# alibaba/open-simulator

Measured on AMD Instinct MI355X. Metric: capacity-plan scenarios/sec (10k pods x ~1k nodes), higher is better.
Workload: dtype u8 score table + u32 (gcd-normalised int64 quantities) + f64 (BalancedAllocation); 1 GPU; BASELINE config 3: 10000 pods x 488..1511 nodes, 1024 node counts x 4 pod orders = 4096 scenarios (4096 per GPU); scenarios_per_gpu=4096, pods=10000, node_pool=1512, kernel=score_table

## Files before the change

__graft_entry__.py:

```python
import os
import subprocess
import sys

ROOT = os.path.dirname(os.path.abspath(__file__))
if ROOT not in sys.path:
    sys.path.insert(0, ROOT)

CSRC = os.path.join(ROOT, "open-simulator_amd", "csrc")
HIP_SOURCES = ["simon_hip.hip", "simon_group.hip", "simon_narrow.hip", "simon_fast.hip", "simon_table.hip", "simon_table_spread.hip", "simon_table_spread2.hip", "simon_table_team4.hip", "simon_table_team4z.hip", "simon_table_rest.hip", "simon_table_rest2.hip", "simon_table_rs.hip", "simon_table_rsz.hip", "simon_table_cls4.hip", "simon_table_lds.hip", "simon_table_restlds.hip", "simon_image.hip", "simon_subset.hip", "simon_wide.hip", "simon_wide_local.hip", "simon_wide_explain.hip"]
HIP_HEADERS = ["simon_device.h", "simon_wide.h", "simon_table.h", "simon_subset.h", "simon_table_assume.inc", os.path.join(ROOT, "include", "simon_hip.h")]
EXTRA_DEPS = {**{f"simon_table_team{n}.hip": ["simon_table.hip"] for n in (4,)}, "simon_table_spread.hip": ["simon_table.hip"], "simon_table_spread2.hip": ["simon_table.hip"], "simon_table_rest.hip": ["simon_table.hip"], "simon_table_rest2.hip": ["simon_table.hip"], "simon_table_rs.hip": ["simon_table.hip"], "simon_table_rsz.hip": ["simon_table.hip"], "simon_table_team4z.hip": ["simon_table.hip"], "simon_table_cls4.hip": ["simon_table.hip"], "simon_table_lds.hip": ["simon_table.hip"], "simon_table_restlds.hip": ["simon_table.hip"], "simon_image.hip": ["simon_table.hip"],
              "simon_wide_local.hip": ["simon_wide.hip"], "simon_wide_explain.hip": ["simon_wide.hip"]}
HIPCC_FLAGS = ["--offload-arch=gfx950", "-O3", "-std=c++17", "-ffp-contract=off", "-fPIC"]


def _stale(target, deps):
    if not os.path.exists(target):
        return True
    t = os.path.getmtime(target)
    return any(os.path.getmtime(d) > t for d in deps)


def _isa_path(src):
    return os.path.join(ROOT, "build", "isa", os.path.basename(src)[:-4] + ".s")


def _spill_scan(hipcc, srcs, hdrs) -> None:
    os.makedirs(os.path.join(ROOT, "build", "isa"), exist_ok=True)
    outs, jobs = [], []
    for src in srcs:
        out = _isa_path(src)
        outs.append(out)
        if _stale(out, [src] + hdrs + [os.path.join(CSRC, d) for d in EXTRA_DEPS.get(os.path.basename(src), [])]):
            jobs.append((src, subprocess.Popen([hipcc, *HIPCC_FLAGS, "--cuda-device-only", "-S", "-o", out, src], stderr=subprocess.DEVNULL)))
    for src, job in jobs:
        if job.wait() != 0:
            raise RuntimeError(f"hipcc -S failed on {src}")
    sys.path.insert(0, os.path.join(ROOT, "profiles"))
    import spill_scan
    bad = []
    for out in outs:
        bad += [(os.path.basename(out),) + f for f in spill_scan.scan(out)[1]]
    if bad:
# ... 68 lines not shown
```

open-simulator_amd/csrc/simon_table.hip:

```cpp
#include "simon_table.h"

#include <algorithm>
#include <type_traits>

#ifdef SIMON_TABLE_PROFILE
#define TPROF_DECL unsigned long long tp_prev = __builtin_readcyclecounter(), tp_acc[24] = {0}; tp_acc[22] = tp_prev - tp_pro0; tp_acc[23] = tp_pro2;
#define TPROF_PROLOGUE_BEGIN const unsigned long long tp_pro0 = __builtin_readcyclecounter(); unsigned long long tp_pro2 = 0;
#define TPROF_TABLE_PASS_BEGIN tp_pro2 = __builtin_readcyclecounter()
#define TPROF_TABLE_PASS_END do { asm volatile("s_waitcnt vmcnt(0) lgkmcnt(0)" ::: "memory"); tp_pro2 = __builtin_readcyclecounter() - tp_pro2; } while (0)
#define TPROF(i) do { const unsigned long long t_ = __builtin_readcyclecounter(); tp_acc[i] += t_ - tp_prev; tp_prev = t_; } while (0)
#define TPROF_WAIT_LDS asm volatile("s_waitcnt lgkmcnt(0)" ::: "memory")
#define TPROF_WAIT_MEM asm volatile("s_waitcnt vmcnt(0)" ::: "memory")
#else
#define TPROF_DECL
#define TPROF_PROLOGUE_BEGIN
#define TPROF_TABLE_PASS_BEGIN do { } while (0)
#define TPROF_TABLE_PASS_END do { } while (0)
#define TPROF(i) do { } while (0)
#define TPROF_WAIT_LDS do { } while (0)
#define TPROF_WAIT_MEM do { } while (0)
#endif

namespace simon {

// ... 252 lines not shown
    const int32_t* __restrict__ orders, const int32_t* __restrict__ perm, const unsigned long long* __restrict__ ws_off,
    int32_t* __restrict__ place_step, unsigned char* ws, const TableScalars sc) {
    GPtr<const TableCold> const cold = gp(cold_);
    GPtr<const int32_t> __restrict__ const ncls = gp(cold->ncls);
    GPtr<const int32_t> __restrict__ const cls_off = gp(cold->cls_off); GPtr<const int32_t> __restrict__ const clsprefix = gp(cold->clsprefix);
    GPtr<const int32_t> __restrict__ const a_pods = gp(cold->a_pods); GPtr<const uint32_t> __restrict__ const i_rq_cpu = gp(cold->i_rq_cpu);
    GPtr<const uint32_t> __restrict__ const i_rq_mem = gp(cold->i_rq_mem); GPtr<const uint32_t> __restrict__ const i_nz_cpu = gp(cold->i_nz_cpu);
    GPtr<const uint32_t> __restrict__ const i_nz_mem = gp(cold->i_nz_mem); GPtr<const int32_t> __restrict__ const i_npods = gp(cold->i_npods);
    const SigRow* __restrict__ const sigs = cold->sigs; const ShapeRow* __restrict__ const shapes = cold->shapes;
    const ScenarioDesc* __restrict__ const scen = cold->scen; GPtr<const uint64_t> __restrict__ const static_mask = gp(cold->static_mask);
    GPtr<const int32_t> __restrict__ const simon_raw = gp(cold->simon_raw);
    extern __shared__ __attribute__((aligned(16))) unsigned char smem[];
    const int Cn = sc.Cn, Cp = sc.Cp, P = sc.P, K = sc.K;
    constexpr int UB = COARSE ? 6 : 4;
    constexpr int UNIT = 1 << UB;
    constexpr unsigned UMASK = UNIT - 1;
    constexpr int KB = COARSE ? 13 : 12;
    constexpr unsigned PMASK = (1u << KB) - 1u;
    static_assert(!REST || COARSE, "the REST path is built on the two-level layout");
    constexpr bool kCls4 = CN2 && !REST && !SPREAD;
#ifdef SIMON_REST_CNT_HBM
    constexpr bool CNT_LDS = !COARSE;
#else
    constexpr bool CNT_LDS = (!COARSE || REST) && !kCls4;
#endif
#ifdef SIMON_TIE_SPECULATE
    constexpr bool TIE_FIRST = false;
#else
    constexpr bool TIE_FIRST = REST || MANY;
#endif
    constexpr bool kStraight = !REST && !SPREAD && !MANY;
    static_assert(!(kStraight && TIE_FIRST), "the straight-line cycle defines the winner's class and record index behind the assume's loads: nothing ahead of them may read dstar / res");
    static_assert(!kStraight || NW == 1, "team mode is SPREAD: a straight-line instantiation has no helper waves");
    constexpr bool kSharedPro = kSharedPrologueTU && !COARSE && !REST && !SPREAD && !MANY && !kCls4 && !RANKED && !LDSWS && NW == 1;
    static_assert(!MANY || (KQ == 2 && COARSE && !CN2 && !LDSX), "MANY = groups of 128 signatures on the two-level layout (since round 6 also under the REST select: its rows and counters are indexed by signature already)");
    constexpr int NG = MANY ? 2 : 0;
    static_assert(!SPREAD || COARSE, "SPREAD is built on the two-level layout");
    constexpr bool RS = REST && SPREAD;
    static_assert(!RS || (!LDSX && !CN2), "REST && SPREAD: <= 64 classes");
    static_assert(!(SPREAD && MANY) || NBQ == 2, "SPREAD with more than 128 signatures: the two-blocks-per-lane instantiations only");
    static_assert(NW == 1 || SPREAD, "team mode exists for the SPREAD instantiations");
    static_assert(!CN2 || (SPREAD && !MANY && !REST) || (REST && !LDSX && !SPREAD) || (!REST && !SPREAD && !COARSE && !MANY && !LDSWS), "CN2 = two node classes per lane in spread_select (<= 128 signatures) or in rest_select (rows in HBM); without rows and walks: 129 .. 256 classes on the one-level layout (simon_table_cls4.hip)");
    constexpr int TABMAX = CN2 ? kSpreadTabMax2 : kSpreadTabMax;
    const TCarve cv = tcarve(K, sc.ni_max, Cn, COARSE, REST, SPREAD ? (sc.NZK | ((sc.static_tables & kStSpreadAff) ? 0x100 : 0) | (NW > 1 ? 0x200 : 0) | (CN2 ? 0x400 : 0)) : -1, kCls4);
    const int TH = SPREAD ? sc.TH : 0, TZ = SPREAD ? sc.TZ : 0, NZK = SPREAD ? sc.NZK : 0;
    signed char* s_zdom = (signed char*)(smem + cv.zdom);
    unsigned short* s_stash = (unsigned short*)(smem + cv.stash);
    int* s_tabi = (int*)(smem + cv.tabi);
    int* s_tab = (int*)(smem + cv.tab);
    int* s_tot = NW > 1 ? (int*)(smem + cv.tab2) : s_tab;
    int* s_xch = (int*)(smem + cv.xch);
    const int M = REST ? sc.M : 0, G = REST ? sc.G : 0, X = REST ? sc.X : 0, NZ = REST ? sc.NZ : 0;
    const int nbp = cv.nbp;
    unsigned short* s_sn = (unsigned short*)(smem + cv.sn);
    int* s_cnt = (int*)(smem + cv.cnt);
    const ShapeRow* s_shape = (const ShapeRow*)(smem + cv.shape);
    auto shape_of = [&](int d) -> ShapeRow {
        if constexpr (kCls4) {
            const double* r = (const double*)(smem + cv.shape) + 4 * d;
            return ShapeRow{r[0], r[1], r[2], r[3], 100.0 * r[2], 100.0 * r[3]};
        } else return s_shape[d];
    };
    int* s_seg = (int*)(smem + cv.seg);
    int* s_tmp = (int*)(smem + cv.tmp);
    int2* s_ext = (int2*)(smem + cv.ext);

// ... 302 lines not shown
    if constexpr (SPREAD) {
        for (int i = tid; i < (NZK > 0 ? NZK : 1) * Cn; i += TT) s_zdom[i] = NZK > 0 ? gp(cold->cls_zdom)[i] : (signed char)0;
        for (size_t i = tid; i < ((size_t)TH * ni + 3) / 4; i += TT) ((unsigned*)g_hrow)[i] = 0u;
        for (int i = tid; i < TZ * 16; i += TT) g_zcnt[i] = 0u;
        for (int i = tid; i < TH; i += TT) g_hmax[i] = 0;
    }
    asm volatile("s_waitcnt vmcnt(0)" ::: "memory");
    if constexpr (NW > 1 || kCls4) __threadfence();
    __syncthreads();
    if constexpr (NW > 1) __threadfence();

    int kk[KQ];
    bool kvalid[KQ];
    double my_req_c[KQ], my_req_m[KQ], my_nz_c[KQ], my_nz_m[KQ];
    bool my_zero[KQ];
    int my_tc[KQ];
    unsigned my_add_c[KQ], my_add_m[KQ], my_addz_c[KQ], my_addz_m[KQ], koff[KQ];
    unsigned my_greq[KQ];
    int my_gnum[KQ];
    unsigned my_dirty = 0;
#pragma unroll
    for (int q = 0; q < KQ; ++q) {
        kvalid[q] = lane + 64 * q < K;
        kk[q] = kvalid[q] ? lane + 64 * q : 0;
        const SigRow r = sigs[kk[q]];
        my_req_c[q] = r.req_c; my_req_m[q] = r.req_m; my_nz_c[q] = r.nz_c; my_nz_m[q] = r.nz_m;
        my_zero[q] = r.flags & 1u;
        if constexpr (kCls4) my_tc[q] = r.cls;
        my_greq[q] = (unsigned)r.pad[0]; my_gnum[q] = kvalid[q] ? r.pad[1] : 0;
        my_add_c[q] = (unsigned)r.req_c; my_add_m[q] = (unsigned)r.req_m;
        my_addz_c[q] = (unsigned)r.nz_c; my_addz_m[q] = (unsigned)r.nz_m;
        koff[q] = (unsigned)kk[q] * KS;
    }
    for (int j = 0; j * 64 + lane < K; ++j) my_dirty |= 1u << j;
    int cb[NBQ], bcls[NBQ], binfo[NBQ];
#pragma unroll
    for (int q = 0; q < NBQ; ++q) {
        const int b = q * 64 + lane;
        cb[q] = (((int)(PMASK >> UB)) - b) << UB;
        bcls[q] = class_of_pos(b < nun ? b * UNIT : 0);
        binfo[q] = (cls_off[bcls[q]] - s_seg[bcls[q]] + 8192) | (bcls[q] << 16);
    }

    auto winner_info = [&](int bw) -> int {
        const int l = bw & 63, h = bw >> 6;
        int info = __builtin_amdgcn_readlane(binfo[0], l);
        if (NBQ > 1) { const int i1 = __builtin_amdgcn_readlane(binfo[NBQ > 1 ? 1 : 0], l); info = h == 1 ? i1 : info; }
        if (NBQ > 2) {
            const int i2 = __builtin_amdgcn_readlane(binfo[NBQ > 2 ? 2 : 0], l), i3 = __builtin_amdgcn_readlane(binfo[NBQ > 3 ? 3 : 0], l);
            info = h == 2 ? i2 : h == 3 ? i3 : info;
        }
        return info;
    };

    auto img_base = [&](GPtr<const TableCold> cc) -> size_t {
        return (size_t)__builtin_amdgcn_readfirstlane(gp(cc->img_slot)[s]) * (size_t)cc->img_stride;
    };
    auto class_term = [&](bool inb, int rawc, int c, int dd) -> int {
        const int lo = wave_min_i32(inb ? rawc : 0x7fffffff);
        const int hi = wave_max_i32(inb ? rawc : (int)0x80000000);
        const int range = hi >= lo ? hi - lo : 0;
        const double rr = range ? 1.0 / (double)range : 0.0;
        int term = (inb && range) ? 2 * (int)__builtin_fma((double)(rawc - lo) * 100.0, rr, 0.5 * rr) : 0;
        GPtr<const TableCold> cc = cold;
        asm volatile("" : "+s"(cc));
        if (sc.static_tables & kStNa) {
            const int v = gp(cc->na_raw)[c * Cn + dd];
            const int mx = wave_max_i32(inb ? v : 0);
            const double r = mx ? 1.0 / (double)mx : 0.0;
            term += (inb && mx) ? (int)__builtin_fma((double)v * 100.0, r, 0.5 * r) : 0;
        }
        if (sc.static_tables & kStTt) {
            const int v = gp(cc->tt_raw)[c * Cn + dd];
            const int mx = wave_max_i32(inb ? v : 0);
            const double r = mx ? 1.0 / (double)mx : 0.0;
            term += inb ? (mx ? 100 - (int)__builtin_fma((double)v * 100.0, r, 0.5 * r) : 100) : 0;
        }
        if (sc.static_tables & kStAdd) term += inb ? gp(cc->add_raw)[c * Cn + dd] : 0;
        if (sc.static_tables & kStImg) term += inb ? (int)gp(cc->img)[img_base(cc) + c * Cn + dd] : 0;
        return term;
    };
    auto class_term2 = [&](bool in0, bool in1, int raw0, int raw1, int c, int d0, int d1, int& t0, int& t1) {
        const int lo = min(wave_min_i32(in0 ? raw0 : 0x7fffffff), wave_min_i32(in1 ? raw1 : 0x7fffffff));
        const int hi = max(wave_max_i32(in0 ? raw0 : (int)0x80000000), wave_max_i32(in1 ? raw1 : (int)0x80000000));
        const int range = hi >= lo ? hi - lo : 0;
        const double rr = range ? 1.0 / (double)range : 0.0;
// ... 929 lines not shown
            const int zd = s_zdom[zst * Cn + dstar];
            L.on = L.on && zd >= 0;
            L.old = g_zcnt[rowt * 16 + (zd >= 0 ? zd : 0)];
        } else {
            L.on = false;
        }
        return L;
    };
    auto spread_count_store = [&](const SpreadLoads& L, int pstar, int dstar, int spv, int spt, int soft_n, int match_n) {
        const int e = lane - soft_n;
        if (e < 0 || e >= match_n || !L.on) return;
        const unsigned mult = ((unsigned)spv >> 16) & 0xFFu;
        const int kindt = spt & 3, rowt = (spt >> 2) & 0x3FFF, zst = (spt >> 16) & 7;
        const unsigned nv = L.old + mult;
        if (kindt == 1) {
            g_hrow[(size_t)rowt * ni + (unsigned)pstar] = (unsigned char)nv;
            if (nv > L.mx) g_hmax[rowt] = (unsigned char)nv;
        } else {
            g_zcnt[rowt * 16 + s_zdom[zst * Cn + dstar]] = nv;
        }
    };

    int unsched = 0;
    int32_t* __restrict__ place = place_step ? place_step + (size_t)s * P : nullptr;

    auto load_chunk = [&](int i0) -> int4 {
        const int idx = i0 + lane;
        if (idx >= P) return make_int4((int)0x80000000, -1, 0x7fffffff, 0);
        const PodRowC r = pods[order[idx]];
        const bool gated_out = segd ? (r.gate >= 0 && gp(cold->rk_rank)[(size_t)s * (size_t)cold->N + r.gate] >= n) : r.gate >= n;
        const bool special = gated_out || r.preset != -1;
        return make_int4(r.sigcls | (special ? (int)0x80000000 : 0), r.preset, r.gate, r.rest);
    };
    int4 nxt = load_chunk(0);
    auto load_spw = [&](int i0) -> int {
        if constexpr (RS) { const int idx = i0 + lane; return idx < P ? gp(cold->sp_word)[order[idx]] : 0; }
        else return 0;
    };
    int nxt_sw = load_spw(0);
    uint4 pos_c = make_uint4(SIMON_POSC(0), SIMON_POSC(1), SIMON_POSC(2), SIMON_POSC(3));
    asm volatile("" : "+v"(pos_c.x), "+v"(pos_c.y), "+v"(pos_c.z), "+v"(pos_c.w));

    for (int i0 = 0; i0 < P; i0 += 64) {
        const int4 cur = nxt;
        nxt = load_chunk(i0 + 64);
        const int cur_sw = nxt_sw;
        if constexpr (RS) nxt_sw = load_spw(i0 + 64);
        int steps = P - i0 < 64 ? P - i0 : 64;
        if constexpr (kStraight) asm volatile("" : "+s"(steps));
        int plreg = -2;
        for (int il = 0; il < steps; ++il) {
        TPROF(0);
        const int pk = __builtin_amdgcn_readlane(cur.x, il);
        const int r_sig = pk & 0x3FF, r_cls = (pk >> 10) & 0x1FFFFF;
        const int rw = (REST || SPREAD) ? __builtin_amdgcn_readlane(cur.w, il) : 0;
        const int sw = RS ? __builtin_amdgcn_readlane(cur_sw, il) : rw;
        const int sp_soft = SPREAD ? (sw & 7) : 0, sp_match = SPREAD ? ((sw >> 3) & 127) : 0, sp_ipa = SPREAD ? ((sw >> 10) & 7) : 0, sp_hard = SPREAD ? ((sw >> 13) & 3) : 0;
        int spv = 0;
        int spt = 0;
        if (SPREAD && __builtin_expect(sw != 0, 0) && lane < sp_soft + sp_match + sp_ipa + sp_hard) {
            const int2 spe = ldg_i2(gp(cold->sp_ent) + (((unsigned)sw >> 15) + lane));
            spv = spe.x; spt = spe.y;
        }
        const int r_gs = REST ? (rw & 63) - 1 : -1, r_xs = REST ? ((rw >> 6) & 63) - 1 : -1, r_nrows = REST ? (rw >> 12) & 63 : 0;
        int rowv = 0;
        if (REST && lane < r_nrows) rowv = gp(cold->xrows)[((unsigned)rw >> 18) + lane];
        unsigned rtv = 0;
        if (REST && AFF && lane < r_nrows && ((unsigned)rowv >> 31)) rtv = g_rowtot[(unsigned)rowv & 0xFFFFu];

        const uint4* const sel_tab = (const uint4*)kSel;
        auto assume = [&](const bool scanned, const bool bound, int& pstar, int& dstar, int& res, const unsigned top, const unsigned (&m16q)[NBQ], const unsigned (&e16q)[NBQ]) __attribute__((always_inline)) {
            if constexpr (kStraight) {
#include "simon_table_assume.inc"
            }
        };
        int res, pstar = -1, dstar = 0;
        unsigned top = 0, m16q[NBQ], e16q[NBQ];
        bool scanned = false, bound = false;
        const bool spread_pod = SPREAD && pk >= 0 && (sp_soft | sp_ipa | sp_hard) != 0;
        if (!lead) {
            res = -2;
        } else if (__builtin_expect(pk < 0, 0)) {
            const int r_preset = __builtin_amdgcn_readlane(cur.y, il), r_gate = __builtin_amdgcn_readlane(cur.z, il);
            GPtr<const TableCold> cc = cold;
            asm volatile("" : "+s"(cc));
            if (segd ? (r_gate >= 0 && __builtin_amdgcn_readfirstlane(gp(cc->rk_rank)[(size_t)s * (size_t)cc->N + r_gate]) >= n) : r_gate >= n) {
                res = -2;
            } else if (r_preset >= 0) {
                bound = true;
                dstar = __builtin_amdgcn_readfirstlane(gp(cc->ncls)[r_preset]);
                const int rk = __builtin_amdgcn_readfirstlane(ranked ? gp(cc->rk_pos)[(size_t)s * (size_t)cc->N + r_preset] : gp(cc->rank)[r_preset]);
                pstar = __builtin_amdgcn_readfirstlane(s_seg[dstar]) + rk;
                res = __builtin_amdgcn_readfirstlane(gp(cc->cls_off)[dstar]) + rk;
            } else {
                const int pin = -2 - r_preset;
                res = -1;
                if (HAS_PIN && (segd ? __builtin_amdgcn_readfirstlane(gp(cc->rk_rank)[(size_t)s * (size_t)cc->N + pin]) < n : pin < n)) {
                    const int dp = __builtin_amdgcn_readfirstlane(gp(cc->ncls)[pin]);
                    const int rk = __builtin_amdgcn_readfirstlane(ranked ? gp(cc->rk_pos)[(size_t)s * (size_t)cc->N + pin] : gp(cc->rank)[pin]);
                    const int pp = __builtin_amdgcn_readfirstlane(s_seg[dp]) + rk;
                    const unsigned char byte = g_tile[tile_blk((unsigned)(pp >> 4)) + (unsigned)r_sig * KS + (unsigned)(pp & 15)];
                    bool clear = true;
                    if (REST && rw != 0) clear = !((__builtin_amdgcn_readfirstlane(excluded(pp >> 4, r_nrows, rowv, r_gs, r_xs, aff_escape(r_nrows, rowv, rtv))) >> (pp & 15)) & 1u);
                    if (byte != 0 && clear) { res = __builtin_amdgcn_readfirstlane(gp(cc->cls_off)[dp]) + rk; pstar = pp; dstar = dp; }
                }
            }
            if constexpr (kStraight) {
                if (pstar >= 0) assume(false, bound, pstar, dstar, res, 0u, m16q, e16q);
            }
        } else if (REST && __builtin_expect(rw != 0, 0) && !(RS && spread_pod)) {
            pstar = rest_select(r_sig, r_cls, r_nrows, rowv, r_gs, r_xs, aff_escape(r_nrows, rowv, rtv), dstar, res);
            TPROF(10);
            if (pstar < 0) res = -1;
        } else if (spread_pod) {
            const int k = r_sig;
            const unsigned dq = (unsigned)__builtin_amdgcn_readlane((int)my_dirty, k & 63);
            if ((dq >> (k >> 6)) & 1u) {
                renormalise(k, r_cls);
                if (lane == (k & 63)) my_dirty &= ~(1u << (k >> 6));
            }
            if constexpr (NW == 1) {
                if constexpr (RS) pstar = spread_select(k, r_cls, sp_soft, sp_match, sp_ipa, sp_hard, spv, spt, dstar, res, r_nrows, rowv, r_gs, r_xs, aff_escape(r_nrows, rowv, rtv));
                else pstar = spread_select(k, r_cls, sp_soft, sp_match, sp_ipa, sp_hard, spv, spt, dstar, res);
                TPROF(18);
                if (pstar < 0) res = -1;
            }
        } else {
            const int k = r_sig;
            const unsigned dq = (unsigned)__builtin_amdgcn_readlane((int)my_dirty, k & 63);
            if (__builtin_expect((dq >> (k >> 6)) & 1u, 0)) {
                renormalise(k, r_cls);
                if (lane == (k & 63)) my_dirty &= ~(1u << (k >> 6));
            }
            int ks = k;
            asm volatile("" : "+s"(ks));
            const unsigned short* srow = s_sum + ks * nbp;
            unsigned key = 0;
#pragma unroll
            for (int q = 0; q < NBQ; ++q) {
                const int b = q * 64 + lane;
                m16q[q] = srow[b < nun ? b : 0];
            }
#pragma unroll
            for (int q = 0; q < NBQ; ++q) {
                const unsigned m16 = m16q[q];
                if constexpr (kStraight) {
                    unsigned e;
                    asm("v_lshrrev_b32 %0, %2, %1" : "=v"(e) : "v"(m16), "n"(UB));
                    e16q[q] = e;
                    unsigned lo;
                    asm("v_and_or_b32 %0, %1, %2, %3" : "=v"(lo) : "v"(m16), "n"(UMASK), "v"(cb[q]));
                    key = max(key, (e << KB) | lo);
                } else {
                    key = max(key, (((m16 << (KB - UB)) & ~PMASK) | (unsigned)cb[q]) | (m16 & UMASK));
                }
            }
            TPROF_WAIT_LDS; TPROF(1);
            key = wave_max_u32(key);
            TPROF(2);
            if (__builtin_expect(key <= PMASK, 0)) {
                res = -1;
            } else {
                pstar = (int)(PMASK - (key & PMASK));
                top = key >> KB;
                scanned = true;
                if constexpr (kStraight) {
                    assume(true, false, pstar, dstar, res, top, m16q, e16q);
                } else {
                    const int info = winner_info(pstar >> UB);
                    dstar = info >> 16;
                    res = (info & 0xFFFF) - 8192 + pstar;
                }
            }
        }
        if constexpr (NW > 1) {
            if (spread_pod) {
                if constexpr (RS) pstar = spread_select(r_sig, r_cls, sp_soft, sp_match, sp_ipa, sp_hard, spv, spt, dstar, res, r_nrows, rowv, r_gs, r_xs, aff_escape(r_nrows, rowv, rtv));
                else pstar = spread_select(r_sig, r_cls, sp_soft, sp_match, sp_ipa, sp_hard, spv, spt, dstar, res);
                TPROF(18);
                if (pstar < 0) res = -1;
            }
        }
        if constexpr (!kStraight) {
            if (lead && pstar >= 0) {
#include "simon_table_assume.inc"
            }
        }
#ifdef SIMON_TABLE_DEBUG
        if (lane == 0) printf("DBG s=%d step=%d sig=%d cls=%d pstar=%d dstar=%d res=%d top=%u ni=%d nblk=%d\n", s, i0 + il, r_sig, r_cls, pstar, dstar, res, top, ni, nblk);
#endif
        if constexpr (kStraight) plreg = llvm_amdgcn_writelane(res, il, plreg);
        else plreg = (il == lane) ? res : plreg;
        }
        unsched += __popcll(__ballot(lane < steps && plreg == -1));
        if (lead && place && lane < steps) place[i0 + lane] = plreg >= 0 ? cls_list[rk_off + (unsigned)plreg] : plreg;
    }

    if (!lead) return;
    long long uc = 0, um = 0;
    for (int p = lane; p < ni; p += 64) { const NodeState st = g_state[p]; uc += st.rq_c; um += st.rq_m; }
    uc = wave_sum_i64(uc);
    um = wave_sum_i64(um);
#ifdef SIMON_TABLE_PROFILE
    if (lane == 0 && cold->prof)
        for (int q = 0; q < 24; ++q) gp(cold->prof)[(size_t)s * 24 + q] = tp_acc[q];
#endif
    if (lane == 0) {
        gp(cold->unscheduled)[s] = unsched;
        gp(cold->used_cpu)[s] = uc * (long long)sc.g_cpu;
        gp(cold->used_mem)[s] = um * (long long)sc.g_mem;
    }
}

hipError_t launch_table_team4(const TableLaunch& a, int n_blocks, size_t lds_bytes, hipStream_t st);
hipError_t launch_table_team_nzeq4(const TableLaunch& a, int n_blocks, size_t lds_bytes, hipStream_t st);
hipError_t launch_table_rs(const TableLaunch& a, int n_blocks, size_t lds_bytes, hipStream_t st);
hipError_t launch_table_rs_nzeq(const TableLaunch& a, int n_blocks, size_t lds_bytes, hipStream_t st);
hipError_t launch_table_spread2(const TableLaunch& a, int n_blocks, size_t lds_bytes, hipStream_t st);
hipError_t launch_table_spread(const TableLaunch& a, int n_blocks, size_t lds_bytes, hipStream_t st);
hipError_t launch_table_lds(const TableLaunch& a, int n_blocks, size_t lds_bytes, hipStream_t st);
hipError_t launch_table_rest2(const TableLaunch& a, int n_blocks, size_t lds_bytes, hipStream_t st);
hipError_t launch_table_rest_lds(const TableLaunch& a, int n_blocks, size_t lds_bytes, hipStream_t st);
hipError_t launch_table_rest(const TableLaunch& a, int n_blocks, size_t lds_bytes, hipStream_t st);
hipError_t launch_table_cls4(const TableLaunch& a, int n_blocks, size_t lds_bytes, hipStream_t st);

template <class Kern>
static hipError_t launch_kernel(Kern kern, const TableLaunch& a, int n_blocks, int waves, size_t lds, hipStream_t st) {
    hipError_t e = hipFuncSetAttribute((const void*)kern, hipFuncAttributeMaxDynamicSharedMemorySize, (int)lds);
    if (e != hipSuccess) return e;
    hipLaunchKernelGGL(kern, dim3(n_blocks), dim3(64 * waves), lds, st, a.cold, a.cls_list, a.pods, a.orders, a.perm, a.ws_off, a.place_step, a.ws, a.sc);
    return hipGetLastError();
}

template <int... Vs> struct OneOf { int v; };
template <class F> static hipError_t with_consts(F&& f) { return f(); }
// ... 267 lines not shown
```

open-simulator_amd/csrc/simon_table_assume.inc:

```
            TPROF(3);
            auto tie_with_other_class = [&]() -> bool {
                bool other = false;
#pragma unroll
                for (int q = 0; q < NBQ; ++q) other |= ((kStraight ? e16q[q] : m16q[q] >> UB) == top) & (bcls[q] != dstar);
                return __ballot(other) != 0;
            };
            auto canonical_first = [&]() -> int {
#ifdef SIMON_TABLE_PROFILE
                tp_acc[7] += 1;
#endif
                unsigned key2 = 0;
                int canon[NBQ];
#pragma unroll
                for (int q = 0; q < NBQ; ++q) {
                    const int pq = (q * 64 + lane) * UNIT + (UNIT - 1) - (int)(m16q[q] & UMASK);
                    const bool tied = (m16q[q] >> UB) == top && q * 64 + lane < nun;
                    if constexpr (LDSX) canon[q] = tied ? (int)sx_canon[pq] : (int)PMASK;
                    else {
                    canon[q] = tied ? cls_list[rk_off + (unsigned)((binfo[q] & 0xFFFF) - 8192 + pq)] : (int)PMASK;
                    if (ranked && tied) canon[q] = gp(cold->rk_rank)[(size_t)s * (size_t)cold->N + canon[q]];
                    }
                }
#pragma unroll
                for (int q = 0; q < NBQ; ++q) {
                    const int pq = (q * 64 + lane) * UNIT + (UNIT - 1) - (int)(m16q[q] & UMASK);
                    if ((m16q[q] >> UB) == top && q * 64 + lane < nun) key2 = max(key2, ((PMASK - (unsigned)canon[q]) << KB) | (unsigned)pq);
                }
                key2 = wave_max_u32(key2);
                return (int)(key2 & PMASK);
            };
            if (TIE_FIRST && scanned && __builtin_expect(tie_with_other_class(), 0)) {
                const int p2 = canonical_first();
                if (p2 != pstar) {
                    pstar = p2;
                    const int info = winner_info(pstar >> UB);
                    dstar = info >> 16;
                    res = (info & 0xFFFF) - 8192 + pstar;
                }
            }
            NodeState* stp = g_state + pstar;
            NodeState st = *stp;
            using RowRef = std::conditional_t<MANY, unsigned char*, unsigned>;
            auto row_ref = [&](unsigned off) -> RowRef { if constexpr (MANY) return g_tile + off; else return off; };
            auto row_vec = [&](RowRef r) -> uint4 { if constexpr (MANY) return *(const uint4*)r; else return *(const uint4*)(g_tile + r); };
            auto row_byte = [&](RowRef r, int i) -> unsigned char& { if constexpr (MANY) return r[i]; else return g_tile[r + (unsigned)i]; };
            auto byte_ref = [&](RowRef r, int i) -> RowRef {
                if constexpr (kStraight) return r + (unsigned)i;
                else return r;
            };
            auto byte_at = [&](RowRef b, int i) -> unsigned char& { if constexpr (kStraight) return g_tile[b]; else return row_byte(b, i); };
            RowRef rowp[KQ], bytep[KQ];
            uint4 T[KQ];
            uint2 F[KQ];
            unsigned oldq[KQ];
#pragma unroll
            for (int q = 0; q < KQ; ++q) {
                rowp[q] = row_ref(tile_blk((unsigned)(pstar >> 4)) + koff[q]);
                T[q] = row_vec(rowp[q]);
                bytep[q] = byte_ref(rowp[q], pstar & 15);
                oldq[q] = byte_at(bytep[q], pstar & 15);
                if (COARSE) F[q] = *(const uint2*)(g_fine + ((unsigned)(pstar >> 6) * (unsigned)K + (unsigned)kk[q]) * 4u);
            }
            constexpr bool kFoldable = COARSE && !REST && HAS_PIN;
            const bool fold = kFoldable && (sc.static_tables & kStFold);
            const unsigned KW = ((unsigned)K + 31u) >> 5;
            unsigned xfold[KQ];
            if constexpr (kFoldable) {
                if (__builtin_expect(fold, 0)) {
// ... 1 lines not shown
                    for (int q = 0; q < KQ; ++q) xfold[q] = gp(cold->foldx)[(unsigned)r_sig * KW + ((unsigned)kk[q] >> 5)];
                }
            }
            unsigned xfg[NG ? NG : 1][KQ];
            RowRef rowg[NG ? NG : 1][KQ];
            uint4 Tg[NG ? NG : 1][KQ];
            uint2 Fg[NG ? NG : 1][KQ];
            unsigned oldg[NG ? NG : 1][KQ];
            int kg[NG ? NG : 1][KQ];
            if constexpr (MANY) {
#pragma unroll
                for (int g = 0; g < NG; ++g) {
                    if (128 * (g + 1) < K) {
#pragma unroll
                        for (int q = 0; q < KQ; ++q) {
                            const int k = 128 * (g + 1) + 64 * q + lane;
                            kg[g][q] = k < K ? k : 0;
                            rowg[g][q] = row_ref(tile_blk((unsigned)(pstar >> 4)) + (unsigned)kg[g][q] * KS);
                            Tg[g][q] = row_vec(rowg[g][q]);
                            oldg[g][q] = row_byte(rowg[g][q], pstar & 15);
                            Fg[g][q] = *(const uint2*)(g_fine + ((unsigned)(pstar >> 6) * (unsigned)K + (unsigned)kg[g][q]) * 4u);
                            if (__builtin_expect(fold, 0)) xfg[g][q] = gp(cold->foldx)[(unsigned)r_sig * KW + ((unsigned)kg[g][q] >> 5)];
                        }
                    }
                }
            }
            uint2 z = make_uint2(0, 0);
            if (!NZEQ) z = g_nz[pstar];
            if constexpr (kStraight) {
                if (scanned) {
                    __builtin_amdgcn_sched_barrier(0);
#pragma unroll
                    for (int q = 0; q < KQ; ++q) asm volatile("" : "+v"(bytep[q]));
                    const int info = winner_info(pstar >> UB);
                    dstar = info >> 16;
                    res = (info & 0xFFFF) - 8192 + pstar;
                }
            }
            if (!TIE_FIRST && scanned && __builtin_expect(tie_with_other_class(), 0)) {
                const int p2 = canonical_first();
                if (p2 != pstar) {
                    pstar = p2;
                    const int info = winner_info(pstar >> UB);
                    dstar = info >> 16;
                    res = (info & 0xFFFF) - 8192 + pstar;
                    stp = g_state + pstar;
                    st = *stp;
#pragma unroll
                    for (int q = 0; q < KQ; ++q) {
                        rowp[q] = row_ref(tile_blk((unsigned)(pstar >> 4)) + koff[q]);
                        T[q] = row_vec(rowp[q]);
                        bytep[q] = byte_ref(rowp[q], pstar & 15);
                        oldq[q] = byte_at(bytep[q], pstar & 15);
                        if (COARSE) F[q] = *(const uint2*)(g_fine + ((unsigned)(pstar >> 6) * (unsigned)K + (unsigned)kk[q]) * 4u);
                    }
                    if (!NZEQ) z = g_nz[pstar];
                }
            }
            const int blk = pstar >> 4, pos = pstar & 15;
            int c15 = 15 - pos;
            if constexpr (kStraight) asm volatile("" : "+s"(c15));
            RestLoads RL{};
            if (REST && __builtin_expect(rw != 0, 0)) RL = rest_assume_load(pstar, r_nrows, rowv, bound ? -1 : r_gs, r_xs);
            uint4 gfa = make_uint4(0, 0, 0, 0), gfb = make_uint4(0, 0, 0, 0);
            unsigned gft = 0;
            int gfc = 0;
            if constexpr (kGpuFoldable) {
                if (__builtin_expect(gfold, 0)) {
                    gfc = g_fc[pstar]; gft = g_ft[pstar];
                    gfa = *(const uint4*)(g_fu + (size_t)pstar * 8); gfb = *(const uint4*)(g_fu + (size_t)pstar * 8 + 4);
                }
            }
            SpreadLoads SPL{0u, 0u, false};
            if (SPREAD && sp_match != 0) SPL = spread_count_load(pstar, dstar, res, spv, spt, sp_soft, sp_match);
            const ShapeRow sh = shape_of(dstar);
            unsigned snq[KQ];
// ... 162 lines not shown
```

Measured before the change: 398,000 scenarios/s.

## Specialise per-pod cycle on active bucket-quad count per scenario

Moves the per-pod scheduling loop into an include file and instantiates it up to three times with a compile-time NQ chosen from the scenario's number of used buckets (nun ≤64, ≤128, or the full NBQ). Scenarios with fewer nodes then scan fewer 64-lane bucket groups per pod: fewer LDS reads, max reductions and readlanes in the hot loop. It also swaps the final 64-bit wave sum for a ds_bpermute butterfly. The cost is larger code size and more instruction-cache pressure from the three loop copies, plus possible register-allocation differences between them.

```diff
diff --git a/__graft_entry__.py b/__graft_entry__.py
--- a/__graft_entry__.py
+++ b/__graft_entry__.py
@@ -8,7 +8,7 @@
 
 CSRC = os.path.join(ROOT, "open-simulator_amd", "csrc")
 HIP_SOURCES = ["simon_hip.hip", "simon_group.hip", "simon_narrow.hip", "simon_fast.hip", "simon_table.hip", "simon_table_spread.hip", "simon_table_spread2.hip", "simon_table_team4.hip", "simon_table_team4z.hip", "simon_table_rest.hip", "simon_table_rest2.hip", "simon_table_rs.hip", "simon_table_rsz.hip", "simon_table_cls4.hip", "simon_table_lds.hip", "simon_table_restlds.hip", "simon_image.hip", "simon_subset.hip", "simon_wide.hip", "simon_wide_local.hip", "simon_wide_explain.hip"]
-HIP_HEADERS = ["simon_device.h", "simon_wide.h", "simon_table.h", "simon_subset.h", "simon_table_assume.inc", os.path.join(ROOT, "include", "simon_hip.h")]
+HIP_HEADERS = ["simon_device.h", "simon_wide.h", "simon_table.h", "simon_subset.h", "simon_table_assume.inc", "simon_table_cycle.inc", os.path.join(ROOT, "include", "simon_hip.h")]
 EXTRA_DEPS = {**{f"simon_table_team{n}.hip": ["simon_table.hip"] for n in (4,)}, "simon_table_spread.hip": ["simon_table.hip"], "simon_table_spread2.hip": ["simon_table.hip"], "simon_table_rest.hip": ["simon_table.hip"], "simon_table_rest2.hip": ["simon_table.hip"], "simon_table_rs.hip": ["simon_table.hip"], "simon_table_rsz.hip": ["simon_table.hip"], "simon_table_team4z.hip": ["simon_table.hip"], "simon_table_cls4.hip": ["simon_table.hip"], "simon_table_lds.hip": ["simon_table.hip"], "simon_table_restlds.hip": ["simon_table.hip"], "simon_image.hip": ["simon_table.hip"],
               "simon_wide_local.hip": ["simon_wide.hip"], "simon_wide_explain.hip": ["simon_wide.hip"]}
 HIPCC_FLAGS = ["--offload-arch=gfx950", "-O3", "-std=c++17", "-ffp-contract=off", "-fPIC"]
diff --git a/open-simulator_amd/csrc/simon_table.hip b/open-simulator_amd/csrc/simon_table.hip
--- a/open-simulator_amd/csrc/simon_table.hip
+++ b/open-simulator_amd/csrc/simon_table.hip
@@ -308,6 +308,7 @@
     constexpr bool kStraight = !REST && !SPREAD && !MANY;
     static_assert(!(kStraight && TIE_FIRST), "the straight-line cycle defines the winner's class and record index behind the assume's loads: nothing ahead of them may read dstar / res");
     static_assert(!kStraight || NW == 1, "team mode is SPREAD: a straight-line instantiation has no helper waves");
+    constexpr bool kPerScenNQ = kStraight && !COARSE && !LDSWS && !kCls4 && !RANKED && NBQ > 1;
     constexpr bool kSharedPro = kSharedPrologueTU && !COARSE && !REST && !SPREAD && !MANY && !kCls4 && !RANKED && !LDSWS && NW == 1;
     static_assert(!MANY || (KQ == 2 && COARSE && !CN2 && !LDSX), "MANY = groups of 128 signatures on the two-level layout (since round 6 also under the REST select: its rows and counters are indexed by signature already)");
     constexpr int NG = MANY ? 2 : 0;
@@ -676,7 +677,7 @@
         my_addz_c[q] = (unsigned)r.nz_c; my_addz_m[q] = (unsigned)r.nz_m;
         koff[q] = (unsigned)kk[q] * KS;
     }
-    for (int j = 0; j * 64 + lane < K; ++j) my_dirty |= 1u << j;
+    if constexpr (!kPerScenNQ) { for (int j = 0; j * 64 + lane < K; ++j) my_dirty |= 1u << j; }
     int cb[NBQ], bcls[NBQ], binfo[NBQ];
 #pragma unroll
     for (int q = 0; q < NBQ; ++q) {
@@ -686,16 +687,18 @@
         binfo[q] = (cls_off[bcls[q]] - s_seg[bcls[q]] + 8192) | (bcls[q] << 16);
     }
 
-    auto winner_info = [&](int bw) -> int {
+    auto winner_info_n = [&](auto nq, int bw) -> int {
+        constexpr int N = decltype(nq)::value;
         const int l = bw & 63, h = bw >> 6;
         int info = __builtin_amdgcn_readlane(binfo[0], l);
-        if (NBQ > 1) { const int i1 = __builtin_amdgcn_readlane(binfo[NBQ > 1 ? 1 : 0], l); info = h == 1 ? i1 : info; }
-        if (NBQ > 2) {
-            const int i2 = __builtin_amdgcn_readlane(binfo[NBQ > 2 ? 2 : 0], l), i3 = __builtin_amdgcn_readlane(binfo[NBQ > 3 ? 3 : 0], l);
+        if (N > 1) { const int i1 = __builtin_amdgcn_readlane(binfo[N > 1 ? 1 : 0], l); info = h == 1 ? i1 : info; }
+        if (N > 2) {
+            const int i2 = __builtin_amdgcn_readlane(binfo[N > 2 ? 2 : 0], l), i3 = __builtin_amdgcn_readlane(binfo[N > 3 ? 3 : 0], l);
             info = h == 2 ? i2 : h == 3 ? i3 : info;
         }
         return info;
     };
+    auto winner_info = [&](int bw) -> int { return winner_info_n(std::integral_constant<int, NBQ>{}, bw); };
 
     auto img_base = [&](GPtr<const TableCold> cc) -> size_t {
         return (size_t)__builtin_amdgcn_readfirstlane(gp(cc->img_slot)[s]) * (size_t)cc->img_stride;
@@ -1691,175 +1694,58 @@
         const bool special = gated_out || r.preset != -1;
         return make_int4(r.sigcls | (special ? (int)0x80000000 : 0), r.preset, r.gate, r.rest);
     };
-    int4 nxt = load_chunk(0);
+    int4 nxt;
+    if constexpr (!kPerScenNQ) nxt = load_chunk(0);
     auto load_spw = [&](int i0) -> int {
         if constexpr (RS) { const int idx = i0 + lane; return idx < P ? gp(cold->sp_word)[order[idx]] : 0; }
         else return 0;
     };
-    int nxt_sw = load_spw(0);
+    int nxt_sw = 0;
+    if constexpr (!kPerScenNQ) nxt_sw = load_spw(0);
     uint4 pos_c = make_uint4(SIMON_POSC(0), SIMON_POSC(1), SIMON_POSC(2), SIMON_POSC(3));
     asm volatile("" : "+v"(pos_c.x), "+v"(pos_c.y), "+v"(pos_c.z), "+v"(pos_c.w));
 
-    for (int i0 = 0; i0 < P; i0 += 64) {
-        const int4 cur = nxt;
-        nxt = load_chunk(i0 + 64);
-        const int cur_sw = nxt_sw;
-        if constexpr (RS) nxt_sw = load_spw(i0 + 64);
-        int steps = P - i0 < 64 ? P - i0 : 64;
-        if constexpr (kStraight) asm volatile("" : "+s"(steps));
-        int plreg = -2;
-        for (int il = 0; il < steps; ++il) {
-        TPROF(0);
-        const int pk = __builtin_amdgcn_readlane(cur.x, il);
-        const int r_sig = pk & 0x3FF, r_cls = (pk >> 10) & 0x1FFFFF;
-        const int rw = (REST || SPREAD) ? __builtin_amdgcn_readlane(cur.w, il) : 0;
-        const int sw = RS ? __builtin_amdgcn_readlane(cur_sw, il) : rw;
-        const int sp_soft = SPREAD ? (sw & 7) : 0, sp_match = SPREAD ? ((sw >> 3) & 127) : 0, sp_ipa = SPREAD ? ((sw >> 10) & 7) : 0, sp_hard = SPREAD ? ((sw >> 13) & 3) : 0;
-        int spv = 0;
-        int spt = 0;
-        if (SPREAD && __builtin_expect(sw != 0, 0) && lane < sp_soft + sp_match + sp_ipa + sp_hard) {
-            const int2 spe = ldg_i2(gp(cold->sp_ent) + (((unsigned)sw >> 15) + lane));
-            spv = spe.x; spt = spe.y;
-        }
-        const int r_gs = REST ? (rw & 63) - 1 : -1, r_xs = REST ? ((rw >> 6) & 63) - 1 : -1, r_nrows = REST ? (rw >> 12) & 63 : 0;
-        int rowv = 0;
-        if (REST && lane < r_nrows) rowv = gp(cold->xrows)[((unsigned)rw >> 18) + lane];
-        unsigned rtv = 0;
-        if (REST && AFF && lane < r_nrows && ((unsigned)rowv >> 31)) rtv = g_rowtot[(unsigned)rowv & 0xFFFFu];
-
-        const uint4* const sel_tab = (const uint4*)kSel;
-        auto assume = [&](const bool scanned, const bool bound, int& pstar, int& dstar, int& res, const unsigned top, const unsigned (&m16q)[NBQ], const unsigned (&e16q)[NBQ]) __attribute__((always_inline)) {
-            if constexpr (kStraight) {
-#include "simon_table_assume.inc"
-            }
-        };
-        int res, pstar = -1, dstar = 0;
-        unsigned top = 0, m16q[NBQ], e16q[NBQ];
-        bool scanned = false, bound = false;
-        const bool spread_pod = SPREAD && pk >= 0 && (sp_soft | sp_ipa | sp_hard) != 0;
-        if (!lead) {
-            res = -2;
-        } else if (__builtin_expect(pk < 0, 0)) {
-            const int r_preset = __builtin_amdgcn_readlane(cur.y, il), r_gate = __builtin_amdgcn_readlane(cur.z, il);
-            GPtr<const TableCold> cc = cold;
-            asm volatile("" : "+s"(cc));
-            if (segd ? (r_gate >= 0 && __builtin_amdgcn_readfirstlane(gp(cc->rk_rank)[(size_t)s * (size_t)cc->N + r_gate]) >= n) : r_gate >= n) {
-                res = -2;
-            } else if (r_preset >= 0) {
-                bound = true;
-                dstar = __builtin_amdgcn_readfirstlane(gp(cc->ncls)[r_preset]);
-                const int rk = __builtin_amdgcn_readfirstlane(ranked ? gp(cc->rk_pos)[(size_t)s * (size_t)cc->N + r_preset] : gp(cc->rank)[r_preset]);
-                pstar = __builtin_amdgcn_readfirstlane(s_seg[dstar]) + rk;
-                res = __builtin_amdgcn_readfirstlane(gp(cc->cls_off)[dstar]) + rk;
+    if constexpr (kPerScenNQ) {
+        if (nun <= 64) {
+            constexpr int NQ = 1;
+#include "simon_table_cycle.inc"
+        } else {
+            if constexpr (NBQ == 4) {
+                if (nun <= 128) {
+                    constexpr int NQ = 2;
+#include "simon_table_cycle.inc"
+                } else {
+                    constexpr int NQ = 4;
+#include "simon_table_cycle.inc"
+                }
             } else {
-                const int pin = -2 - r_preset;
-                res = -1;
-                if (HAS_PIN && (segd ? __builtin_amdgcn_readfirstlane(gp(cc->rk_rank)[(size_t)s * (size_t)cc->N + pin]) < n : pin < n)) {
-                    const int dp = __builtin_amdgcn_readfirstlane(gp(cc->ncls)[pin]);
-                    const int rk = __builtin_amdgcn_readfirstlane(ranked ? gp(cc->rk_pos)[(size_t)s * (size_t)cc->N + pin] : gp(cc->rank)[pin]);
-                    const int pp = __builtin_amdgcn_readfirstlane(s_seg[dp]) + rk;
-                    const unsigned char byte = g_tile[tile_blk((unsigned)(pp >> 4)) + (unsigned)r_sig * KS + (unsigned)(pp & 15)];
-                    bool clear = true;
-                    if (REST && rw != 0) clear = !((__builtin_amdgcn_readfirstlane(excluded(pp >> 4, r_nrows, rowv, r_gs, r_xs, aff_escape(r_nrows, rowv, rtv))) >> (pp & 15)) & 1u);
-                    if (byte != 0 && clear) { res = __builtin_amdgcn_readfirstlane(gp(cc->cls_off)[dp]) + rk; pstar = pp; dstar = dp; }
-                }
-            }
-            if constexpr (kStraight) {
-                if (pstar >= 0) assume(false, bound, pstar, dstar, res, 0u, m16q, e16q);
-            }
-        } else if (REST && __builtin_expect(rw != 0, 0) && !(RS && spread_pod)) {
-            pstar = rest_select(r_sig, r_cls, r_nrows, rowv, r_gs, r_xs, aff_escape(r_nrows, rowv, rtv), dstar, res);
-            TPROF(10);
-            if (pstar < 0) res = -1;
-        } else if (spread_pod) {
-            const int k = r_sig;
-            const unsigned dq = (unsigned)__builtin_amdgcn_readlane((int)my_dirty, k & 63);
-            if ((dq >> (k >> 6)) & 1u) {
-                renormalise(k, r_cls);
-                if (lane == (k & 63)) my_dirty &= ~(1u << (k >> 6));
-            }
-            if constexpr (NW == 1) {
-                if constexpr (RS) pstar = spread_select(k, r_cls, sp_soft, sp_match, sp_ipa, sp_hard, spv, spt, dstar, res, r_nrows, rowv, r_gs, r_xs, aff_escape(r_nrows, rowv, rtv));
-                else pstar = spread_select(k, r_cls, sp_soft, sp_match, sp_ipa, sp_hard, spv, spt, dstar, res);
-                TPROF(18);
-                if (pstar < 0) res = -1;
-            }
-        } else {
-            const int k = r_sig;
-            const unsigned dq = (unsigned)__builtin_amdgcn_readlane((int)my_dirty, k & 63);
-            if (__builtin_expect((dq >> (k >> 6)) & 1u, 0)) {
-                renormalise(k, r_cls);
-                if (lane == (k & 63)) my_dirty &= ~(1u << (k >> 6));
-            }
-            int ks = k;
-            asm volatile("" : "+s"(ks));
-            const unsigned short* srow = s_sum + ks * nbp;
-            unsigned key = 0;
-#pragma unroll
-            for (int q = 0; q < NBQ; ++q) {
-                const int b = q * 64 + lane;
-                m16q[q] = srow[b < nun ? b : 0];
-            }
-#pragma unroll
-            for (int q = 0; q < NBQ; ++q) {
-                const unsigned m16 = m16q[q];
-                if constexpr (kStraight) {
-                    unsigned e;
-                    asm("v_lshrrev_b32 %0, %2, %1" : "=v"(e) : "v"(m16), "n"(UB));
-                    e16q[q] = e;
-                    unsigned lo;
-                    asm("v_and_or_b32 %0, %1, %2, %3" : "=v"(lo) : "v"(m16), "n"(UMASK), "v"(cb[q]));
-                    key = max(key, (e << KB) | lo);
-                } else {
-                    key = max(key, (((m16 << (KB - UB)) & ~PMASK) | (unsigned)cb[q]) | (m16 & UMASK));
-                }
-            }
-            TPROF_WAIT_LDS; TPROF(1);
-            key = wave_max_u32(key);
-            TPROF(2);
-            if (__builtin_expect(key <= PMASK, 0)) {
-                res = -1;
-            } else {
-                pstar = (int)(PMASK - (key & PMASK));
-                top = key >> KB;
-                scanned = true;
-                if constexpr (kStraight) {
-                    assume(true, false, pstar, dstar, res, top, m16q, e16q);
-                } else {
-                    const int info = winner_info(pstar >> UB);
-                    dstar = info >> 16;
-                    res = (info & 0xFFFF) - 8192 + pstar;
-                }
-            }
-        }
-        if constexpr (NW > 1) {
-            if (spread_pod) {
-                if constexpr (RS) pstar = spread_select(r_sig, r_cls, sp_soft, sp_match, sp_ipa, sp_hard, spv, spt, dstar, res, r_nrows, rowv, r_gs, r_xs, aff_escape(r_nrows, rowv, rtv));
-                else pstar = spread_select(r_sig, r_cls, sp_soft, sp_match, sp_ipa, sp_hard, spv, spt, dstar, res);
-                TPROF(18);
-                if (pstar < 0) res = -1;
-            }
-        }
-        if constexpr (!kStraight) {
-            if (lead && pstar >= 0) {
-#include "simon_table_assume.inc"
-            }
-        }
-#ifdef SIMON_TABLE_DEBUG
-        if (lane == 0) printf("DBG s=%d step=%d sig=%d cls=%d pstar=%d dstar=%d res=%d top=%u ni=%d nblk=%d\n", s, i0 + il, r_sig, r_cls, pstar, dstar, res, top, ni, nblk);
-#endif
-        if constexpr (kStraight) plreg = llvm_amdgcn_writelane(res, il, plreg);
-        else plreg = (il == lane) ? res : plreg;
-        }
-        unsched += __popcll(__ballot(lane < steps && plreg == -1));
-        if (lead && place && lane < steps) place[i0 + lane] = plreg >= 0 ? cls_list[rk_off + (unsigned)plreg] : plreg;
+                constexpr int NQ = NBQ;
+#include "simon_table_cycle.inc"
+            }
+        }
+    } else {
+        constexpr int NQ = NBQ;
+#include "simon_table_cycle.inc"
     }
 
     if (!lead) return;
     long long uc = 0, um = 0;
     for (int p = lane; p < ni; p += 64) { const NodeState st = g_state[p]; uc += st.rq_c; um += st.rq_m; }
-    uc = wave_sum_i64(uc);
-    um = wave_sum_i64(um);
+    if constexpr (kPerScenNQ) {
+        auto sum64 = [&](long long v) -> long long {
+            for (int off = 32; off > 0; off >>= 1) {
+                const int a = (lane ^ off) << 2;
+                const unsigned lo = (unsigned)__builtin_amdgcn_ds_bpermute(a, (int)(unsigned)v), hi = (unsigned)__builtin_amdgcn_ds_bpermute(a, (int)(unsigned)((unsigned long long)v >> 32));
+                v += (long long)(((unsigned long long)hi << 32) | lo);
+            }
+            return v;
+        };
+        uc = sum64(uc);
+        um = sum64(um);
+    } else {
+        uc = wave_sum_i64(uc);
+        um = wave_sum_i64(um);
+    }
 #ifdef SIMON_TABLE_PROFILE
     if (lane == 0 && cold->prof)
         for (int q = 0; q < 24; ++q) gp(cold->prof)[(size_t)s * 24 + q] = tp_acc[q];
diff --git a/open-simulator_amd/csrc/simon_table_assume.inc b/open-simulator_amd/csrc/simon_table_assume.inc
--- a/open-simulator_amd/csrc/simon_table_assume.inc
+++ b/open-simulator_amd/csrc/simon_table_assume.inc
@@ -2,7 +2,7 @@
             auto tie_with_other_class = [&]() -> bool {
                 bool other = false;
 #pragma unroll
-                for (int q = 0; q < NBQ; ++q) other |= ((kStraight ? e16q[q] : m16q[q] >> UB) == top) & (bcls[q] != dstar);
+                for (int q = 0; q < NQ; ++q) other |= ((kStraight ? e16q[q] : m16q[q] >> UB) == top) & (bcls[q] != dstar);
                 return __ballot(other) != 0;
             };
             auto canonical_first = [&]() -> int {
@@ -10,9 +10,9 @@
                 tp_acc[7] += 1;
 #endif
                 unsigned key2 = 0;
-                int canon[NBQ];
-#pragma unroll
-                for (int q = 0; q < NBQ; ++q) {
+                int canon[NQ];
+#pragma unroll
+                for (int q = 0; q < NQ; ++q) {
                     const int pq = (q * 64 + lane) * UNIT + (UNIT - 1) - (int)(m16q[q] & UMASK);
                     const bool tied = (m16q[q] >> UB) == top && q * 64 + lane < nun;
                     if constexpr (LDSX) canon[q] = tied ? (int)sx_canon[pq] : (int)PMASK;
@@ -22,7 +22,7 @@
                     }
                 }
 #pragma unroll
-                for (int q = 0; q < NBQ; ++q) {
+                for (int q = 0; q < NQ; ++q) {
                     const int pq = (q * 64 + lane) * UNIT + (UNIT - 1) - (int)(m16q[q] & UMASK);
                     if ((m16q[q] >> UB) == top && q * 64 + lane < nun) key2 = max(key2, ((PMASK - (unsigned)canon[q]) << KB) | (unsigned)pq);
                 }
@@ -33,7 +33,7 @@
                 const int p2 = canonical_first();
                 if (p2 != pstar) {
                     pstar = p2;
-                    const int info = winner_info(pstar >> UB);
+                    const int info = winner_info_n(std::integral_constant<int, NQ>{}, pstar >> UB);
                     dstar = info >> 16;
                     res = (info & 0xFFFF) - 8192 + pstar;
                 }
@@ -101,7 +101,7 @@
                     __builtin_amdgcn_sched_barrier(0);
 #pragma unroll
                     for (int q = 0; q < KQ; ++q) asm volatile("" : "+v"(bytep[q]));
-                    const int info = winner_info(pstar >> UB);
+                    const int info = winner_info_n(std::integral_constant<int, NQ>{}, pstar >> UB);
                     dstar = info >> 16;
                     res = (info & 0xFFFF) - 8192 + pstar;
                 }
@@ -110,7 +110,7 @@
                 const int p2 = canonical_first();
                 if (p2 != pstar) {
                     pstar = p2;
-                    const int info = winner_info(pstar >> UB);
+                    const int info = winner_info_n(std::integral_constant<int, NQ>{}, pstar >> UB);
                     dstar = info >> 16;
                     res = (info & 0xFFFF) - 8192 + pstar;
                     stp = g_state + pstar;
diff --git a/open-simulator_amd/csrc/simon_table_cycle.inc b/open-simulator_amd/csrc/simon_table_cycle.inc
--- /dev/null
+++ b/open-simulator_amd/csrc/simon_table_cycle.inc
@@ -0,0 +1,159 @@
+    if constexpr (kPerScenNQ) {
+        nxt = load_chunk(0); nxt_sw = load_spw(0);
+        for (int j = 0; j * 64 + lane < K; ++j) my_dirty |= 1u << j;
+        asm volatile("" : "+v"(my_dirty));
+    }
+    for (int i0 = 0; i0 < P; i0 += 64) {
+        const int4 cur = nxt;
+        nxt = load_chunk(i0 + 64);
+        const int cur_sw = nxt_sw;
+        if constexpr (RS) nxt_sw = load_spw(i0 + 64);
+        int steps = P - i0 < 64 ? P - i0 : 64;
+        if constexpr (kStraight) asm volatile("" : "+s"(steps));
+        int plreg = -2;
+        for (int il = 0; il < steps; ++il) {
+        TPROF(0);
+        const int pk = __builtin_amdgcn_readlane(cur.x, il);
+        const int r_sig = pk & 0x3FF, r_cls = (pk >> 10) & 0x1FFFFF;
+        const int rw = (REST || SPREAD) ? __builtin_amdgcn_readlane(cur.w, il) : 0;
+        const int sw = RS ? __builtin_amdgcn_readlane(cur_sw, il) : rw;
+        const int sp_soft = SPREAD ? (sw & 7) : 0, sp_match = SPREAD ? ((sw >> 3) & 127) : 0, sp_ipa = SPREAD ? ((sw >> 10) & 7) : 0, sp_hard = SPREAD ? ((sw >> 13) & 3) : 0;
+        int spv = 0;
+        int spt = 0;
+        if (SPREAD && __builtin_expect(sw != 0, 0) && lane < sp_soft + sp_match + sp_ipa + sp_hard) {
+            const int2 spe = ldg_i2(gp(cold->sp_ent) + (((unsigned)sw >> 15) + lane));
+            spv = spe.x; spt = spe.y;
+        }
+        const int r_gs = REST ? (rw & 63) - 1 : -1, r_xs = REST ? ((rw >> 6) & 63) - 1 : -1, r_nrows = REST ? (rw >> 12) & 63 : 0;
+        int rowv = 0;
+        if (REST && lane < r_nrows) rowv = gp(cold->xrows)[((unsigned)rw >> 18) + lane];
+        unsigned rtv = 0;
+        if (REST && AFF && lane < r_nrows && ((unsigned)rowv >> 31)) rtv = g_rowtot[(unsigned)rowv & 0xFFFFu];
+
+        const uint4* const sel_tab = (const uint4*)kSel;
+        auto assume = [&](const bool scanned, const bool bound, int& pstar, int& dstar, int& res, const unsigned top, const unsigned (&m16q)[NQ], const unsigned (&e16q)[NQ]) __attribute__((always_inline)) {
+            if constexpr (kStraight) {
+#include "simon_table_assume.inc"
+            }
+        };
+        int res, pstar = -1, dstar = 0;
+        unsigned top = 0, m16q[NQ], e16q[NQ];
+        bool scanned = false, bound = false;
+        const bool spread_pod = SPREAD && pk >= 0 && (sp_soft | sp_ipa | sp_hard) != 0;
+        if (!lead) {
+            res = -2;
+        } else if (__builtin_expect(pk < 0, 0)) {
+            const int r_preset = __builtin_amdgcn_readlane(cur.y, il), r_gate = __builtin_amdgcn_readlane(cur.z, il);
+            GPtr<const TableCold> cc = cold;
+            asm volatile("" : "+s"(cc));
+            if (segd ? (r_gate >= 0 && __builtin_amdgcn_readfirstlane(gp(cc->rk_rank)[(size_t)s * (size_t)cc->N + r_gate]) >= n) : r_gate >= n) {
+                res = -2;
+            } else if (r_preset >= 0) {
+                bound = true;
+                dstar = __builtin_amdgcn_readfirstlane(gp(cc->ncls)[r_preset]);
+                const int rk = __builtin_amdgcn_readfirstlane(ranked ? gp(cc->rk_pos)[(size_t)s * (size_t)cc->N + r_preset] : gp(cc->rank)[r_preset]);
+                pstar = __builtin_amdgcn_readfirstlane(s_seg[dstar]) + rk;
+                res = __builtin_amdgcn_readfirstlane(gp(cc->cls_off)[dstar]) + rk;
+            } else {
+                const int pin = -2 - r_preset;
+                res = -1;
+                if (HAS_PIN && (segd ? __builtin_amdgcn_readfirstlane(gp(cc->rk_rank)[(size_t)s * (size_t)cc->N + pin]) < n : pin < n)) {
+                    const int dp = __builtin_amdgcn_readfirstlane(gp(cc->ncls)[pin]);
+                    const int rk = __builtin_amdgcn_readfirstlane(ranked ? gp(cc->rk_pos)[(size_t)s * (size_t)cc->N + pin] : gp(cc->rank)[pin]);
+                    const int pp = __builtin_amdgcn_readfirstlane(s_seg[dp]) + rk;
+                    const unsigned char byte = g_tile[tile_blk((unsigned)(pp >> 4)) + (unsigned)r_sig * KS + (unsigned)(pp & 15)];
+                    bool clear = true;
+                    if (REST && rw != 0) clear = !((__builtin_amdgcn_readfirstlane(excluded(pp >> 4, r_nrows, rowv, r_gs, r_xs, aff_escape(r_nrows, rowv, rtv))) >> (pp & 15)) & 1u);
+                    if (byte != 0 && clear) { res = __builtin_amdgcn_readfirstlane(gp(cc->cls_off)[dp]) + rk; pstar = pp; dstar = dp; }
+                }
+            }
+            if constexpr (kStraight) {
+                if (pstar >= 0) assume(false, bound, pstar, dstar, res, 0u, m16q, e16q);
+            }
+        } else if (REST && __builtin_expect(rw != 0, 0) && !(RS && spread_pod)) {
+            pstar = rest_select(r_sig, r_cls, r_nrows, rowv, r_gs, r_xs, aff_escape(r_nrows, rowv, rtv), dstar, res);
+            TPROF(10);
+            if (pstar < 0) res = -1;
+        } else if (spread_pod) {
+            const int k = r_sig;
+            const unsigned dq = (unsigned)__builtin_amdgcn_readlane((int)my_dirty, k & 63);
+            if ((dq >> (k >> 6)) & 1u) {
+                renormalise(k, r_cls);
+                if (lane == (k & 63)) my_dirty &= ~(1u << (k >> 6));
+            }
+            if constexpr (NW == 1) {
+                if constexpr (RS) pstar = spread_select(k, r_cls, sp_soft, sp_match, sp_ipa, sp_hard, spv, spt, dstar, res, r_nrows, rowv, r_gs, r_xs, aff_escape(r_nrows, rowv, rtv));
+                else pstar = spread_select(k, r_cls, sp_soft, sp_match, sp_ipa, sp_hard, spv, spt, dstar, res);
+                TPROF(18);
+                if (pstar < 0) res = -1;
+            }
+        } else {
+            const int k = r_sig;
+            const unsigned dq = (unsigned)__builtin_amdgcn_readlane((int)my_dirty, k & 63);
+            if (__builtin_expect((dq >> (k >> 6)) & 1u, 0)) {
+                renormalise(k, r_cls);
+                if (lane == (k & 63)) my_dirty &= ~(1u << (k >> 6));
+            }
+            int ks = k;
+            asm volatile("" : "+s"(ks));
+            const unsigned short* srow = s_sum + ks * nbp;
+            unsigned key = 0;
+#pragma unroll
+            for (int q = 0; q < NQ; ++q) {
+                const int b = q * 64 + lane;
+                m16q[q] = srow[b < nun ? b : 0];
+            }
+#pragma unroll
+            for (int q = 0; q < NQ; ++q) {
+                const unsigned m16 = m16q[q];
+                if constexpr (kStraight) {
+                    unsigned e;
+                    asm("v_lshrrev_b32 %0, %2, %1" : "=v"(e) : "v"(m16), "n"(UB));
+                    e16q[q] = e;
+                    unsigned lo;
+                    asm("v_and_or_b32 %0, %1, %2, %3" : "=v"(lo) : "v"(m16), "n"(UMASK), "v"(cb[q]));
+                    key = max(key, (e << KB) | lo);
+                } else {
+                    key = max(key, (((m16 << (KB - UB)) & ~PMASK) | (unsigned)cb[q]) | (m16 & UMASK));
+                }
+            }
+            TPROF_WAIT_LDS; TPROF(1);
+            key = wave_max_u32(key);
+            TPROF(2);
+            if (__builtin_expect(key <= PMASK, 0)) {
+                res = -1;
+            } else {
+                pstar = (int)(PMASK - (key & PMASK));
+                top = key >> KB;
+                scanned = true;
+                if constexpr (kStraight) {
+                    assume(true, false, pstar, dstar, res, top, m16q, e16q);
+                } else {
+                    const int info = winner_info(pstar >> UB);
+                    dstar = info >> 16;
+                    res = (info & 0xFFFF) - 8192 + pstar;
+                }
+            }
+        }
+        if constexpr (NW > 1) {
+            if (spread_pod) {
+                if constexpr (RS) pstar = spread_select(r_sig, r_cls, sp_soft, sp_match, sp_ipa, sp_hard, spv, spt, dstar, res, r_nrows, rowv, r_gs, r_xs, aff_escape(r_nrows, rowv, rtv));
+                else pstar = spread_select(r_sig, r_cls, sp_soft, sp_match, sp_ipa, sp_hard, spv, spt, dstar, res);
+                TPROF(18);
+                if (pstar < 0) res = -1;
+            }
+        }
+        if constexpr (!kStraight) {
+            if (lead && pstar >= 0) {
+#include "simon_table_assume.inc"
+            }
+        }
+#ifdef SIMON_TABLE_DEBUG
+        if (lane == 0) printf("DBG s=%d step=%d sig=%d cls=%d pstar=%d dstar=%d res=%d top=%u ni=%d nblk=%d\n", s, i0 + il, r_sig, r_cls, pstar, dstar, res, top, ni, nblk);
+#endif
+        if constexpr (kStraight) plreg = llvm_amdgcn_writelane(res, il, plreg);
+        else plreg = (il == lane) ? res : plreg;
+        }
+        unsched += __popcll(__ballot(lane < steps && plreg == -1));
+        if (lead && place && lane < steps) place[i0 + lane] = plreg >= 0 ? cls_list[rk_off + (unsigned)plreg] : plreg;
+    }
```

Measured after the change: 406,800 scenarios/s (median of 6 runs). 2.2% higher.
